# wildjames/lfit_python

Hardware: AMD Instinct MI355X
Metric: walker ln_prob evals/sec (300-pt phase, complex BS) at 1/2/4/8 MI355X (higher is better)
Workload: dtype f64

## Files before the change

cpu_baseline/lfg_cpu.cpp:

```cpp
#include <omp.h>
#include <stdint.h>
#include <stdlib.h>

#include <algorithm>
#include <cmath>
#include <vector>

#include "lfg.h"
#include "lfg_cpu.h"
#include "lfg_device.hpp"
#include "lfg_tables.hpp"

using namespace lfg;

namespace {

constexpr int U_WD = NWD / 2, U_DISC = NDISC / 2, U_DON = NDONOR / 4;

struct Pair {
    Roche R;
    double s, c, rwd_a, rdisc_a, reff, rcal, ulimb, dexp, L, upk, umax, lnpk, exp1, exp2;
    double bsx, bsy, caz, saz, nb0, nb1, nb2, bden, fis, phi0, wdf, df, sf, rsf;
    double inc;
};
// ... 69 lines not shown
    G.bden = p[11] + (1.0 - p[11]) * std::fmax(std::fabs(st_) * G.s + ct_ * G.c, 0.0);
    G.fis = p[11];
    G.phi0 = p[13];
    G.ulimb = p[7];
    G.dexp = p[12];
    G.L = p[9] * R.xl1;
    G.reff = eggleton(R.q);
    const double sce = G.s * std::cos(PI * p[5]);
    G.rcal = std::sqrt(1.0 - sce * sce);
    G.wdf = p[0]; G.df = p[1]; G.sf = p[2]; G.rsf = p[3];
    G.inc = inc;
    return ST_OK;
}

struct Tables {
    double a[NWD + NDISC], b[NWD + NDISC], w[NWD + NDISC];
    int wd[NWD + NDISC];
    double sa[NBS], sb[NBS], sw[NBS];
    double dv[NDONOR][3], dcen[NDONOR], dhw[NDONOR];
    double dnorm;
};

#ifdef LFC_COUNT
static unsigned long long g_cnt[4 + 3 * 8];
extern "C" void lfc_counts(unsigned long long* o) { for (int i = 0; i < 4 + 24; ++i) o[i] = g_cnt[i]; }
static unsigned long long g_ucost[U_WD + U_DISC + NBS];
extern "C" void lfc_ucost(unsigned long long* o) { for (int i = 0; i < U_WD + U_DISC + NBS; ++i) { o[i] = g_ucost[i]; g_ucost[i] = 0; } }
static void count_pair(const int* cost, int n)
{
    unsigned long long ls = 0, cm = 0, nc = 0;
    for (int k = 0; k < n; k += 64) {
        int m = 0;
        for (int i = k; i < std::min(n, k + 64); ++i) {
            m = std::max(m, cost[i]);
            ls += cost[i];
            const int reg = i < U_WD ? 0 : (i < U_WD + U_DISC ? 1 : 2);
#pragma omp atomic
            g_ucost[i] += cost[i];
#pragma omp atomic
            g_cnt[4 + reg * 8 + std::min(cost[i], 7)] += 1;
        }
        cm += m; ++nc;
    }
#pragma omp atomic
    g_cnt[0] += n;
#pragma omp atomic
    g_cnt[1] += ls;
#pragma omp atomic
    g_cnt[2] += nc;
#pragma omp atomic
    g_cnt[3] += cm;
}
static unsigned long long g_cnt2[5];
extern "C" void lfc_counts2(unsigned long long* o) { for (int i = 0; i < 5; ++i) o[i] = g_cnt2[i]; }
static void count2(int i, unsigned long long v)
{
#pragma omp atomic
    g_cnt2[i] += v;
}
#define LFC_NIT int nit[3] = {0, 0, 0}; bool fb = false; double gs[2] = {0.0, 0.0};
#define LFC_NITARGS , &fb, nit, gs
#if LFC_COST_MODE == 1
#define LFC_COST(v) cost[v] = nit[0] / 1000
#else
#define LFC_COST(v) cost[v] = nit[0] % 1000 + std::max(nit[1], nit[2]) + (fb ? 30 : 0); count2(0, nit[0] / 1000); count2(1, fb)
#endif
static std::vector<double> g_ab;
extern "C" long lfc_dump(double* o, long n)
{
    const long m = std::min<long>(n, long(g_ab.size()));
    for (long i = 0; i < m; ++i) o[i] = g_ab[i];
    g_ab.clear();
    return m;
}
#define LFC_AB(a, b) do { _Pragma("omp critical") { g_ab.push_back(a); g_ab.push_back(b); g_gs.push_back(gs[0]); g_gs.push_back(gs[1]); } } while (0)
static std::vector<double> g_gs;
extern "C" long lfc_dump_guess(double* o, long n)
{
    const long m = std::min<long>(n, long(g_gs.size()));
    for (long i = 0; i < m; ++i) o[i] = g_gs[i];
    g_gs.clear();
    return m;
}
#else
#define LFC_NIT
#define LFC_NITARGS
#define LFC_COST(v)
#define LFC_AB(a, b)
#endif

void elements(const Pair& G, Tables& T)
{
#ifdef LFC_COUNT
    int cost[U_WD + U_DISC + NBS] = {0};
#endif
    const Roche& R = G.R;
    const double s = G.s, c = G.c;
    const double twd = TWO_PI * ((1.0 - G.ulimb) * 0.5 + G.ulimb / 3.0);
    const double td = TWO_PI * (disc_boundary(NDISC_R, G) - disc_boundary(0, G));
    int k = 0;
    for (int u = 0; u < U_WD + U_DISC; ++u) {
        double Px, Py, Pz, wgt;
        bool isw = u < U_WD;
        if (isw) {
            const int ir = wd_ring_of(u);
            const double rc = kWdRc[ir], mu0 = kWdMu0[ir], cp = kWdCos[u], sp = kWdSin[u];
            Px = G.rwd_a * (-rc * sp * c + mu0 * s);
            Py = G.rwd_a * (rc * cp);
            Pz = G.rwd_a * (rc * sp * s + mu0 * c);
            wgt = std::fma(kWdA[ir], 1.0 - G.ulimb, kWdB[ir] * G.ulimb) / twd;
        } else {
            const int uu = u - U_WD, ir = uu / (NDISC_AZ / 2), j = uu - ir * (NDISC_AZ / 2);
            const double rc = G.rwd_a + (ir + 0.5) * ((G.rdisc_a - G.rwd_a) / NDISC_R);
            Px = rc * kDiscCos[j];
            Py = rc * kDiscSin[j];
            Pz = 0.0;
            wgt = (TWO_PI / NDISC_AZ) * (disc_boundary(ir + 1, G) - disc_boundary(ir, G)) / td;
        }
        double a, b;
        LFC_NIT
        element_interval_fast(R, Px, Py, Pz, s, c, G.rcal, G.reff, a, b LFC_NITARGS);
        LFC_COST(u);
        LFC_AB(a, b);
        T.a[k] = a; T.b[k] = b; T.w[k] = wgt; T.wd[k] = isw; ++k;
        const bool ecl = a < b;
        T.a[k] = ecl ? -b : 1.0; T.b[k] = ecl ? -a : -1.0; T.w[k] = wgt; T.wd[k] = isw; ++k;
    }
    double tot = 0.0;
    for (int j = 0; j < NBS; ++j) {
        const double uk = (j + 0.5) * (G.umax / NBS);
        T.sw[j] = std::exp(G.exp1 * std::log(uk) - std::pow(uk, G.exp2) - G.lnpk);
        tot += T.sw[j];
        const double off = G.L * (uk - G.upk);
        LFC_NIT
        element_interval_fast(R, std::fma(off, G.caz, G.bsx), std::fma(off, G.saz, G.bsy), 0.0, s, c, G.rcal, G.reff,
                              T.sa[j], T.sb[j] LFC_NITARGS);
        LFC_COST(U_WD + U_DISC + j);
        LFC_AB(T.sa[j], T.sb[j]);
    }
#ifdef LFC_COUNT
    count_pair(cost, U_WD + U_DISC + NBS);
#endif
    for (int j = 0; j < NBS; ++j) T.sw[j] /= tot;
    double dn = 0.0;
    for (int uu = 0; uu < U_DON; ++uu) {
        const int it = uu / (NDONOR_P / 4), ip = uu - it * (NDONOR_P / 4);
        const double dx = -kDonCt[it], dy = kDonSt[it] * kDonCp[ip], dz = kDonSt[it] * kDonSp[ip];
        double lo = 0.0, hi = R.Rs, r = G.reff, gx, gy, gz;
        if (!(r > lo && r < hi)) r = 0.5 * hi;
#if LFG_F32_OPEN && LFG_F32_ROOT_STEPS > 0
        r = root_open32<LFG_F32_ROOT_STEPS>(R, dx, dy, dz, hi, r);
#endif
#ifdef LFC_COUNT
        count2(2, 1);
        count2(4, LFG_F32_OPEN ? LFG_F32_ROOT_STEPS : 0);
#endif
        for (int itr = 0; itr < ROOT_MAXIT; ++itr) {
#ifdef LFC_COUNT
            count2(3, 1);
#endif
            const double f = rpot_grad(R, std::fma(r, dx, 1.0), r * dy, r * dz, gx, gy, gz) - R.pl1;
            const double df = gx * dx + gy * dy + gz * dz;
            if (f > 0.0) hi = r; else lo = r;
            if (df > 0.0 && std::fabs(f / df) <= ROOT_LAST) { r -= f / df; break; }
            double rn = (df > 0.0) ? r - f / df : 0.5 * (lo + hi);
            if (!(rn > lo && rn < hi)) rn = 0.5 * (lo + hi);
// ... 430 lines not shown
```

cpu_baseline/shim/hip/hip_runtime.h:

```cpp
#pragma once
#include <algorithm>
#include <cmath>
#define __device__
#define __host__
#define __global__
#define __constant__
#define __forceinline__ inline
#define __noinline__
#define __builtin_amdgcn_rsq(x) (1.0 / std::sqrt(x))
#define __builtin_amdgcn_rcp(x) (1.0 / (x))
#define __builtin_amdgcn_rsqf(x) (1.0f / std::sqrt(float(x)))
#define __builtin_amdgcn_rcpf(x) (1.0f / float(x))
using std::max;
using std::min;
inline double rsqrt(double x) { return 1.0 / std::sqrt(x); }
inline float rsqrtf(float x) { return 1.0f / std::sqrt(x); }
```

lfit_python_amd/csrc/lfg_device.hpp:

```cpp
#pragma once
#include <hip/hip_runtime.h>
#include <math.h>

#include "lfg_stream_table.h"

namespace lfg {

constexpr double PI = 3.14159265358979323846;
constexpr double TWO_PI = 6.28318530717958647693;
constexpr double DEG = PI / 180.0;
constexpr double LN2 = 0.69314718055994530942;

constexpr double RAY_TOL = 1e-13;
constexpr int RAY_MAXIT = 100;
constexpr double TH_TOL = 1e-13;
constexpr int ROOT_MAXIT = 100;
constexpr double ROOT_LAST = 1e-9;
constexpr int MIN_MAXIT = 100;
constexpr double BS_TAIL = 16.0;
constexpr double STREAM_DELTA = 1e-2;
constexpr double STREAM_KAPPA_FINE = 0.15 / 32.0;
constexpr double STREAM_DTMAX_FINE = 0.15 / 32.0;
constexpr int STREAM_MAXSTEP_FINE = 128000;
constexpr double DISC_MAX_A = 0.46;
constexpr double AZ_SLOPE = 80.0;
constexpr double DPHI_TOL = 1e-6;

constexpr int NWD_RINGS = 10;
constexpr int NWD = 400;
constexpr int NDISC_R = 20;
constexpr int NDISC_AZ = 50;
constexpr int NDISC = 1000;
constexpr int NBS = 100;
constexpr int NDONOR_T = 20;
constexpr int NDONOR_P = 20;
constexpr int NDONOR = 400;
constexpr int NEL = NWD + NDISC + NBS;
constexpr int NALL = NEL + NDONOR;

enum Status { ST_OK = 0, ST_BAD_Q = 1, ST_BAD_DPHI = 2, ST_BAD_GEOMETRY = 3,
              ST_BAD_STREAM = 4, ST_BAD_ARGS = 5 };

enum Geo {
    G_Q, G_CA, G_CB, G_MU, G_XL1, G_PL1, G_RS, G_RS2,
    G_S, G_C, G_INC, G_RWD, G_RDISC, G_REFF, G_ULIMB, G_DEXP,
    G_BSX, G_BSY, G_BSVX, G_BSVY, G_L, G_UPK, G_UMAX, G_LNPK,
    G_EXP1, G_EXP2, G_CAZ, G_SAZ, G_NB0, G_NB1, G_NB2, G_BDEN,
    G_FIS, G_PHI0, G_WDF, G_DF, G_SF, G_RSF, G_RPRIOR, G_RCAL,
    G_RPRIOR_BS,
    G_GP_AIN, G_GP_AOUT, G_GP_LAM, G_GP_DCP, G_GP_OK,
    G_GP_DPHI, G_GP_RWD,
    G_COUNT
};
static_assert(G_COUNT <= 48, "LFG_NGEO");

struct Roche {
    double q, cA, cB, mu, xl1, pl1, Rs, Rs2;
};

__device__ __forceinline__ double rsqrt_pos(double x)
{
    const double y = __builtin_amdgcn_rsq(x);
    const double e = fma(-x * y, y, 1.0);
    return fma(y * e, fma(e, 0.375, 0.5), y);
}

__device__ __forceinline__ double rcp_fast(double x)
{
    const double y = __builtin_amdgcn_rcp(x);
    return fma(y, fma(-x, y, 1.0), y);
}

__device__ __forceinline__ double rcp_step(double x)
{
    return __builtin_amdgcn_rcp(x);
}

__device__ __forceinline__ double rpot(const Roche& R, double x, double y, double z)
{
    const double dx = x - 1.0;
    const double xc = x - R.mu;
    return -R.cA * rsqrt(x * x + y * y + z * z) - R.cB * rsqrt(dx * dx + y * y + z * z)
           - xc * xc - y * y;
}

__device__ __forceinline__ double rpot_grad(const Roche& R, double x, double y, double z, double& gx, double& gy,
                                            double& gz)
// ... 195 lines not shown
    const double Dm = (cosD <= -1.0) ? PI : acos(cosD);
    const double lo = thc - Dm, hi = thc + Dm;

    double tw = -1.0, g, dg;
    bool chord = g_eval(R, Px, Py, Pz, s, c, thc, tw, g, dg);
    if (!chord) return false;
    double thi = thc;
    if (!(g < 0.0)) {
        bool found = false, have = false;
        double th = thc, pth = 0.0, pdg = 0.0, mlo = lo, mhi = hi;
        for (int it = 0; it < MIN_MAXIT; ++it) {
            if (chord) {
                if (g < 0.0) { found = true; thi = th; break; }
                if (dg > 0.0) mhi = th; else mlo = th;
            } else {
                if (th < thc) mlo = th; else mhi = th;
            }
            double tn = (chord && have && dg != pdg) ? th - dg * (th - pth) / (dg - pdg)
                                                     : 0.5 * (mlo + mhi);
            if (!(tn > mlo && tn < mhi)) tn = 0.5 * (mlo + mhi);
            if (fabs(tn - th) <= TH_TOL) break;
            if (chord) { pth = th; pdg = dg; have = true; }
            th = tn;
            chord = g_eval(R, Px, Py, Pz, s, c, th, tw, g, dg);
        }
        if (!found) return false;
    }
    double de;
    const double ce = (sqrt(fmax(uu - Reff * Reff, 0.0)) - c * uz) / (s * uxy);
    de = (ce > -1.0 && ce < 1.0) ? acos(ce) : 0.5 * Dm;
    double twi = tw, two = tw;
    const double thin = theta_root(R, Px, Py, Pz, s, c, lo, thi, true, thc - de, twi);
    const double thout = theta_root(R, Px, Py, Pz, s, c, thi, hi, false, thc + de, two);
    a = thin * (1.0 / TWO_PI);
    b = thout * (1.0 / TWO_PI);
    return true;
}

struct ConePt {
    double phi, gth, F2, eHe, etHe, ethHeth, gtt, dX2;
};

__device__ __forceinline__ void cone_point(const Roche& R, double Px, double Py, double Pz, double s,
                                           double c, double cs, double sn, double t, ConePt& o)
{
    const double ex = s * cs, ey = -s * sn;
    const double x = fma(t, ex, Px), y = fma(t, ey, Py), z = fma(t, c, Pz);
    const double r1s = x * x + y * y + z * z;
    const double ir1 = rsqrt_pos(r1s), ir1s = ir1 * ir1;
    const double dx = x - 1.0;
    const double r2s = dx * dx + y * y + z * z;
    const double ir2 = rsqrt_pos(r2s), ir2s = ir2 * ir2;
    const double i1 = R.cA * ir1s * ir1, i2 = R.cB * ir2s * ir2, i12 = i1 + i2;
    const double xm = x - R.mu;
    o.phi = -R.cA * ir1 - R.cB * ir2 - xm * xm - y * y;
    const double gx = i1 * x + i2 * dx - 2.0 * xm;
    const double gy = (i12 - 2.0) * y;
    const double gz = i12 * z;
    const double p1 = x * ex + y * ey + z * c, p2 = p1 - ex;
    const double q1 = x * ey - y * ex, q2 = q1 - ey;
    const double k1 = 3.0 * i1 * ir1s, k2 = 3.0 * i2 * ir2s;
    const double s2 = ex * ex + ey * ey;
    o.F2 = gx * ex + gy * ey + gz * c;
    o.gth = gx * ey - gy * ex;
    o.eHe = i12 - k1 * p1 * p1 - k2 * p2 * p2 - 2.0 * s2;
    o.etHe = -k1 * p1 * q1 - k2 * p2 * q2;
    o.ethHeth = i12 * s2 - k1 * q1 * q1 - k2 * q2 * q2 - 2.0 * s2;
    o.gtt = -(gx * ex + gy * ey);
    o.dX2 = r2s;
}

__device__ __forceinline__ void rotate(double& cs, double& sn, double d)
{
    const double d2 = d * d;
    const double sd = d * (1.0 - d2 * (1.0 / 6.0) * (1.0 - d2 * (1.0 / 20.0) * (1.0 - d2 * (1.0 / 42.0) *
                                                                              (1.0 - d2 * (1.0 / 72.0)))));
    const double cd = 1.0 - d2 * 0.5 * (1.0 - d2 * (1.0 / 12.0) * (1.0 - d2 * (1.0 / 30.0) *
                                                                    (1.0 - d2 * (1.0 / 56.0) * (1.0 - d2 * (1.0 / 90.0)))));
    const double c2 = cs * cd - sn * sd;
    sn = fma(sn, cd, cs * sd);
    cs = c2;
}

#ifndef LFG_TH_LAST
#define LFG_TH_LAST 1e-6
#endif
#ifndef LFG_T_LAST
#define LFG_T_LAST 3e-5
#endif
constexpr double TH_LAST = LFG_TH_LAST;
constexpr double T_LAST = LFG_T_LAST;

struct Tan {
    double th, cs, sn, t;
    int st;
};

template <bool HALLEY = false>
__device__ __forceinline__ void tangency_step(const Roche& R, double Px, double Py, double Pz, double s, double c,
                                              bool ingress, Tan& T, bool halley = true)
{
    ConePt o;
    cone_point(R, Px, Py, Pz, s, c, T.cs, T.sn, T.t, o);
    const double F1 = o.phi - R.pl1;
    const double J11 = T.t * o.gth;
    const double J21 = T.t * o.etHe + o.gth, J22 = o.eHe;
    const double iJ22 = rcp_step(J22);
    const double dt0 = -o.F2 * iJ22;
    const double F1m = fma(0.5 * o.F2, dt0, F1);
    const double den = fma(J21, dt0, J11);
    const bool bad = !(J22 != 0.0) || !(den != 0.0);
    const double iden = rcp_step(den);
    double dth = -F1m * iden;
    if (HALLEY && halley) {
        const double g2 = fma(T.t, fma(T.t, o.ethHeth, o.gtt), -J21 * J21 * iJ22);
        const double h = 0.5 * dth * g2 * iden;
        if (fabs(h) < 0.5) dth = dth * rcp_step(1.0 + h);
    }
    dth = fmin(fmax(dth, -0.05), 0.05);
    const double dt = fma(-J21 * iJ22, dth, dt0);
    T.th += dth;
    T.t += dt;
    const bool conv = fabs(dth) <= TH_LAST && fabs(dt) <= T_LAST;
    const bool good = J22 > 0.0 && ((J11 < 0.0) == ingress) && T.t > 0.0 && o.dX2 < R.Rs2;
    rotate(T.cs, T.sn, dth);
    T.st = bad ? -1 : (conv ? (good ? 1 : -1) : 0);
}

__device__ inline bool tangency(const Roche& R, double Px, double Py, double Pz, double s, double c,
                                bool ingress, double& th, double cs, double sn, double& t, int* nit = nullptr)
{
    Tan T{th, cs, sn, t, 0};
    for (int it = 0; it < 16 && T.st == 0; ++it) {
        if (nit) ++*nit;
        tangency_step(R, Px, Py, Pz, s, c, ingress, T);
    }
    th = T.th;
    t = T.t;
    return T.st == 1;
}

__device__ inline void tangency_pair(const Roche& R, double Px, double Py, double Pz, double s, double c, Tan& A,
                                     Tan& B, int* nit = nullptr, bool halleyA = true, bool halleyB = true)
{
    tangency_step<true>(R, Px, Py, Pz, s, c, true, A, halleyA);
    tangency_step<true>(R, Px, Py, Pz, s, c, false, B, halleyB);
    if (nit) { nit[0] += 1; nit[1] += 1; }
    if (A.st != 0 && B.st != 0) return;
    for (int it = 1; it < 16; ++it) {
        Tan A2 = A, B2 = B;
        tangency_step(R, Px, Py, Pz, s, c, true, A2);
        tangency_step(R, Px, Py, Pz, s, c, false, B2);
        if (nit) { nit[0] += (A.st == 0); nit[1] += (B.st == 0); }
        if (A.st == 0) A = A2;
        if (B.st == 0) B = B2;
        if (A.st != 0 && B.st != 0) break;
    }
}

__device__ __forceinline__ void ray_min_prestep(const Roche& R, double Px, double Py, double Pz, double s, double c,
                                                double icb, Tan& T)
{
    const double ex = s * T.cs, ey = -s * T.sn;
    const double x = fma(T.t, ex, Px), y = fma(T.t, ey, Py), z = fma(T.t, c, Pz);
    const double ir1 = rsqrt_pos(x * x + y * y + z * z), ir1s = ir1 * ir1;
    const double eX = x * ex + y * ey + z * c;
    const double i1 = R.cA * ir1s * ir1;
    const double slope = fma(i1, eX, -2.0 * fma(x - R.mu, ex, y * ey));
    const double curv = fma(i1, fma(-3.0 * eX * eX, ir1s, 1.0), icb);
    T.t -= slope * rcp_fast(curv);
}

#ifndef LFG_F32_OPEN
#define LFG_F32_OPEN 1
#endif
#ifndef LFG_F32_STEPS
#define LFG_F32_STEPS 2
#endif
#ifndef LFG_F32_NEWTON_AFTER
#define LFG_F32_NEWTON_AFTER 1
#endif
#ifndef LFG_F32_ROOT_STEPS
#define LFG_F32_ROOT_STEPS 0
#endif

#if LFG_F32_OPEN
constexpr float F32_OPEN_MIN_WIDTH = 0.03f;
#ifdef __HIP__
typedef float F2 __attribute__((ext_vector_type(2)));
#else
struct F2 {
    float x, y;
};
inline F2 operator+(F2 a, F2 b) { return F2{a.x + b.x, a.y + b.y}; }
inline F2 operator-(F2 a, F2 b) { return F2{a.x - b.x, a.y - b.y}; }
inline F2 operator*(F2 a, F2 b) { return F2{a.x * b.x, a.y * b.y}; }
inline F2 operator-(F2 a) { return F2{-a.x, -a.y}; }
#endif
__device__ __forceinline__ F2 f2(float a) { return F2{a, a}; }
__device__ __forceinline__ F2 f2_rsq(F2 a) { return F2{__builtin_amdgcn_rsqf(a.x), __builtin_amdgcn_rsqf(a.y)}; }
__device__ __forceinline__ F2 f2_rcp(F2 a) { return F2{__builtin_amdgcn_rcpf(a.x), __builtin_amdgcn_rcpf(a.y)}; }

template <int N>
__device__ __forceinline__ void tangency_open32(const Roche& R, double Px, double Py, double Pz, double s, double c,
                                                double Rcal, Tan& A, Tan& B, bool& okA, bool& okB)
{
    float dA, dB, tA, tB;
    okA = okB = true;
    {
        const float cA = float(R.cA), cB = float(R.cB), mu = float(R.mu), pl1 = float(R.pl1);
        const F2 px = f2(float(Px)), py = f2(float(Py)), pz = f2(float(Pz)), sf = f2(float(s)), cf = f2(float(c));
        const float rc = float(Rcal);
        const F2 icb = f2(cB * __builtin_amdgcn_rcpf(rc * rc * rc)) - f2(2.0f) * sf * sf;
        F2 cs{float(A.cs), float(B.cs)}, sn{float(A.sn), float(B.sn)}, t{float(A.t), float(B.t)};
        F2 sum = f2(0.0f);
        {
            const F2 ex = sf * cs, ey = -(sf * sn);
            const F2 x = t * ex + px, y = t * ey + py, z = t * cf + pz;
            const F2 ir1 = f2_rsq(x * x + y * y + z * z), ir1s = ir1 * ir1;
            const F2 eX = x * ex + y * ey + z * cf;
            const F2 i1 = f2(cA) * ir1s * ir1;
            const F2 slope = i1 * eX - f2(2.0f) * ((x - f2(mu)) * ex + y * ey);
            const F2 curv = i1 * (f2(1.0f) - f2(3.0f) * eX * eX * ir1s) + icb;
            t = t - slope * f2_rcp(curv);
        }
#pragma unroll
        for (int k = 0; k < N; ++k) {
            const F2 ex = sf * cs, ey = -(sf * sn);
            const F2 x = t * ex + px, y = t * ey + py, z = t * cf + pz;
            const F2 yz = y * y + z * z;
            const F2 ir1 = f2_rsq(x * x + yz), ir1s = ir1 * ir1;
            const F2 dx = x - f2(1.0f);
            const F2 ir2 = f2_rsq(dx * dx + yz), ir2s = ir2 * ir2;
            const F2 i1 = f2(cA) * ir1s * ir1, i2 = f2(cB) * ir2s * ir2, i12 = i1 + i2;
            const F2 xm = x - f2(mu);
            const F2 F1 = -(f2(cA) * ir1) - f2(cB) * ir2 - xm * xm - y * y - f2(pl1);
            const F2 gx = i1 * x + i2 * dx - f2(2.0f) * xm;
            const F2 gy = (i12 - f2(2.0f)) * y;
            const F2 gz = i12 * z;
            const F2 p1 = x * ex + y * ey + z * cf, p2 = p1 - ex;
            const F2 q1 = x * ey - y * ex, q2 = q1 - ey;
            const F2 k1 = f2(3.0f) * i1 * ir1s, k2 = f2(3.0f) * i2 * ir2s;
            const F2 s2 = ex * ex + ey * ey;
            const F2 Ft = gx * ex + gy * ey + gz * cf;
            const F2 gth = gx * ey - gy * ex;
            const F2 J22 = i12 - k1 * p1 * p1 - k2 * p2 * p2 - f2(2.0f) * s2;
            const F2 etHe = -(k1 * p1 * q1) - k2 * p2 * q2;
            const F2 J11 = t * gth, J21 = t * etHe + gth;
            const F2 iJ22 = f2_rcp(J22);
            const F2 dt0 = -(Ft * iJ22);
            const F2 F1m = f2(0.5f) * Ft * dt0 + F1;
            const F2 iden = f2_rcp(J21 * dt0 + J11);
            F2 dth = -(F1m * iden);
            if (k == 0) {
                const F2 ethHeth = i12 * s2 - k1 * q1 * q1 - k2 * q2 * q2 - f2(2.0f) * s2;
                const F2 gtt = -(gx * ex + gy * ey);
                const F2 g2 = t * (t * ethHeth + gtt) - J21 * J21 * iJ22;
                const F2 h = f2(0.5f) * dth * g2 * iden;
                const F2 dh = dth * f2_rcp(f2(1.0f) + h);
                dth = F2{fabsf(h.x) < 0.5f ? dh.x : dth.x, fabsf(h.y) < 0.5f ? dh.y : dth.y};
            }
            okA = okA && J22.x > 0.0f && fabsf(dth.x) <= 0.05f;
            okB = okB && J22.y > 0.0f && fabsf(dth.y) <= 0.05f;
            t = t + (dt0 - J21 * iJ22 * dth);
            sum = sum + dth;
            const F2 d2 = dth * dth;
            const F2 sd = dth * (f2(1.0f) - d2 * f2(1.0f / 6.0f) * (f2(1.0f) - d2 * f2(1.0f / 20.0f)));
            const F2 cd = f2(1.0f) - d2 * f2(0.5f) * (f2(1.0f) - d2 * f2(1.0f / 12.0f) *
                                                                  (f2(1.0f) - d2 * f2(1.0f / 30.0f)));
            const F2 c2 = cs * cd - sn * sd;
            sn = sn * cd + cs * sd;
            cs = c2;
        }
        const bool wide = float(B.th - A.th) + (sum.y - sum.x) >= F32_OPEN_MIN_WIDTH;
        okA = okA && wide && fabsf(sum.x) <= 0.05f && t.x > 0.0f && t.x < 3.0e38f;
        okB = okB && wide && fabsf(sum.y) <= 0.05f && t.y > 0.0f && t.y < 3.0e38f;
        dA = okA ? sum.x : 0.0f;
        dB = okB ? sum.y : 0.0f;
        tA = t.x;
        tB = t.y;
    }
    A.th += double(dA);
    B.th += double(dB);
    rotate(A.cs, A.sn, double(dA));
    rotate(B.cs, B.sn, double(dB));
    A.t = double(tA);
    B.t = double(tB);
    if (!(okA && okB)) {
        const double icb = R.cB / (Rcal * Rcal * Rcal) - 2.0 * s * s;
        for (int k = 0; k < 2; ++k) {
            Tan& T = k ? B : A;
            if (k ? okB : okA) continue;
            T.t = s * ((1.0 - Px) * T.cs + Py * T.sn) - Pz * c;
            ray_min_prestep(R, Px, Py, Pz, s, c, icb, T);
        }
    }
}

template <int N>
__device__ __forceinline__ double root_open32(const Roche& R, double dx, double dy, double dz, double hi, double r0)
{
    const float cA = float(R.cA), cB = float(R.cB), mu = float(R.mu), pl1 = float(R.pl1);
    const float ax = float(dx), ay = float(dy), az = float(dz), top = float(hi);
    float r = float(r0);
    bool ok = true;
#pragma unroll
    for (int k = 0; k < N; ++k) {
        const float x = fmaf(r, ax, 1.0f), y = r * ay, z = r * az, x1 = r * ax;
        const float yz = y * y + z * z;
        const float ir1 = __builtin_amdgcn_rsqf(x * x + yz), ir2 = __builtin_amdgcn_rsqf(x1 * x1 + yz);
        const float i1 = cA * ir1 * ir1 * ir1, i2 = cB * ir2 * ir2 * ir2;
        const float xm = x - mu;
        const float f = -cA * ir1 - cB * ir2 - xm * xm - y * y - pl1;
        const float gx = i1 * x + i2 * x1 - 2.0f * xm, gy = (i1 + i2 - 2.0f) * y, gz = (i1 + i2) * z;
        const float df = gx * ax + gy * ay + gz * az;
        r -= f * __builtin_amdgcn_rcpf(df);
        ok = ok && df > 0.0f && r > 0.0f && r < top;
    }
    return ok ? double(r) : r0;
}
#endif

__device__ inline int cone_exists(const Roche& R, double Px, double Py, double Pz, double s, double c,
                                  double cs, double sn, double t, int* nit = nullptr)
{
    for (int it = 0; it < 16; ++it) {
        if (nit) ++*nit;
        ConePt o;
        cone_point(R, Px, Py, Pz, s, c, cs, sn, t, o);
        if (o.phi < R.pl1) return (o.dX2 < R.Rs2) ? 1 : -1;
        const double Gth = t * o.gth, Gt = o.F2;
        const double Htt = o.eHe, Hht = o.gth + t * o.etHe, Hhh = t * t * o.ethHeth + t * o.gtt;
        const double det = Hhh * Htt - Hht * Hht;
        if (!(Hhh > 0.0 && Htt > 0.0 && det > 0.0)) return -1;
        const double idet = rcp_fast(det);
        double dth = -(Htt * Gth - Hht * Gt) * idet;
        double dt = -(Hhh * Gt - Hht * Gth) * idet;
        const double big = fmax(fabs(dth), fabs(dt));
        if (big > 0.05) {
            dth *= 0.05 / big;
            dt *= 0.05 / big;
        }
        t += dt;
        if (fabs(dth) <= 1e-12 && fabs(dt) <= 1e-12) return 0;
        rotate(cs, sn, dth);
    }
    return -1;
}

__device__ inline bool element_interval_fast(const Roche& R, double Px, double Py, double Pz, double s,
                                             double c, double Rcal, double Reff, double& a, double& b,
                                             bool* fallback = nullptr, int* nit = nullptr, double* guess = nullptr)
{
    const double ux = 1.0 - Px, uy = -Py, uz = -Pz;
    const double uxy2 = ux * ux + uy * uy;
    const double uu = uxy2 + uz * uz;
    if (uu > R.Rs2 && uxy2 > 0.0 && s > 0.0) {
        const double iuxy = rsqrt(uxy2), uxy = uxy2 * iuxy;
        const double cosD = (sqrt(uu - R.Rs2) - c * uz) * iuxy / s;
        if (!(cosD < 1.0)) { a = 1.0; b = -1.0; return false; }
        const double cc = ux * iuxy, sc = -uy * iuxy;
        const double tc = s * uxy + uz * c;
        int ex;
        {
            const double ex0 = s * cc, ey0 = -s * sc;
            const double x = fma(tc, ex0, Px), y = fma(tc, ey0, Py), z = fma(tc, c, Pz);
            const double dx = x - 1.0, xm = x - R.mu;
            const double r2s = dx * dx + y * y + z * z;
            const double phi = -R.cA * rsqrt_pos(x * x + y * y + z * z) - R.cB * rsqrt_pos(r2s) - xm * xm - y * y;
            if (phi < R.pl1 && r2s < R.Rs2) {
                ex = 1;
                if (nit) ++nit[0];
            } else {
                ex = cone_exists(R, Px, Py, Pz, s, c, cc, sc, tc, nit);
            }
        }
        if (ex == 0) { a = 1.0; b = -1.0; return false; }
        if (ex == 1) {
            const double ce = (sqrt(fmax(uu - Rcal * Rcal, 0.0)) - c * uz) * iuxy / s;
            if (ce > -1.0 && ce < 1.0) {
                const double se = sqrt(1.0 - ce * ce);
                const double thc = atan2(-uy, ux), de = acos(ce);
                double ci = cc * ce + sc * se, si = sc * ce - cc * se;
                double co = cc * ce - sc * se, so = sc * ce + cc * se;
                Tan In{thc - de, ci, si, s * (ux * ci - uy * si) + uz * c, 0};
                Tan Out{thc + de, co, so, s * (ux * co - uy * so) + uz * c, 0};
                if (guess) { guess[0] = In.th; guess[1] = Out.th; }
#if LFG_F32_OPEN
                bool openIn, openOut;
                tangency_open32<LFG_F32_STEPS>(R, Px, Py, Pz, s, c, Rcal, In, Out, openIn, openOut);
                if (nit) nit[0] += 1000 * LFG_F32_STEPS;
                const bool hIn = !(LFG_F32_NEWTON_AFTER && openIn), hOut = !(LFG_F32_NEWTON_AFTER && openOut);
#else
                {
                    const double icb = R.cB / (Rcal * Rcal * Rcal) - 2.0 * s * s;
                    for (Tan* T : {&In, &Out}) ray_min_prestep(R, Px, Py, Pz, s, c, icb, *T);
                }
#endif
#if LFG_F32_OPEN
                tangency_pair(R, Px, Py, Pz, s, c, In, Out, nit ? nit + 1 : nullptr, hIn, hOut);
#else
                tangency_pair(R, Px, Py, Pz, s, c, In, Out, nit ? nit + 1 : nullptr);
#endif
                const double cin = In.cs * cc + In.sn * sc, cout = Out.cs * cc + Out.sn * sc;
                if (In.st == 1 && Out.st == 1 && In.th < Out.th && cin > cosD && cout > cosD) {
                    a = In.th * (1.0 / TWO_PI);
                    b = Out.th * (1.0 / TWO_PI);
                    return true;
                }
            }
        }
    }
    if (fallback) *fallback = true;
    return element_interval(R, Px, Py, Pz, s, c, Reff, a, b);
}

__device__ inline int findphi(const Roche& R, double inc_deg, double& dphi);

__device__ inline int findphi_fast(const Roche& R, double inc_deg, double& dphi)
{
    double s, c;
    sincos(inc_deg * DEG, &s, &c);
    const double cosD = sqrt(1.0 - R.Rs2) / s;
    if (s > 0.0 && cosD < 1.0) {
        const double Dm = acos(cosD);
        const double R0 = eggleton(R.q);
        const double c0 = sqrt(1.0 - R0 * R0) / s;
        double th = (c0 < 1.0) ? acos(c0) : 0.5 * Dm;
        double sn, cs;
        sincos(th, &sn, &cs);
        double t = s * cs;
        if (tangency(R, 0.0, 0.0, 0.0, s, c, false, th, cs, sn, t) && th > 0.0 && th < Dm) {
            dphi = th / PI;
            return ST_OK;
        }
    }
    return findphi(R, inc_deg, dphi);
}

__device__ inline int findphi(const Roche& R, double inc_deg, double& dphi)
{
    const double i = inc_deg * DEG;
    double s, c;
    sincos(i, &s, &c);
    dphi = 0.0;
    const double cosD = sqrt(1.0 - R.Rs2) / s;
    if (!(s > 0.0) || cosD >= 1.0) return ST_BAD_DPHI;
    const double Dm = acos(cosD);
    double tw = -1.0, g, dg;
    g_eval(R, 0.0, 0.0, 0.0, s, c, 0.0, tw, g, dg);
    if (!(g < 0.0)) return ST_BAD_DPHI;
    const double th = theta_root(R, 0.0, 0.0, 0.0, s, c, 0.0, Dm, false, 0.5 * Dm, tw);
    dphi = th / PI;
    return ST_OK;
}

__device__ inline bool h_eval(const Roche& R, double cth, double sth, double c,
                              double& tw, double& h, double& dh)
{
    const double s = sqrt(1.0 - c * c);
    const double ex = s * cth, ey = -s * sth;
    double fm;
    if (!ray_min(R, 0.0, 0.0, 0.0, ex, ey, c, tw, fm)) { h = 1.0; dh = 0.0; return false; }
    double gx, gy, gz;
    rgrad(R, tw * ex, tw * ey, tw * c, gx, gy, gz);
    h = fm - R.pl1;
    const double r = c / s;
    dh = tw * (gx * (-r * cth) + gy * (r * sth) + gz);
    return true;
}

__device__ inline int findi(const Roche& R, double dphi, double& inc_deg)
{
    if (!(dphi > 0.0) || !(dphi < 0.5)) return ST_BAD_DPHI;
    const double the = PI * dphi;
    double sth, cth;
    sincos(the, &sth, &cth);
    if (!(cth > 0.0)) return ST_BAD_DPHI;
    const double smin = sqrt(1.0 - R.Rs2) / cth;
    if (smin >= 1.0) return ST_BAD_DPHI;
    const double cmax = sqrt(1.0 - smin * smin);
    double tw = -1.0, h, dh;
    h_eval(R, cth, sth, 0.0, tw, h, dh);
    if (!(h < 0.0)) return ST_BAD_DPHI;
    double lo = 0.0, hi = cmax, c = 0.5 * cmax;
    for (int it = 0; it < ROOT_MAXIT; ++it) {
        h_eval(R, cth, sth, c, tw, h, dh);
        if (h > 0.0) hi = c; else lo = c;
        double cn = (dh != 0.0) ? c - h / dh : 0.5 * (lo + hi);
        if (!(cn > lo && cn < hi)) cn = 0.5 * (lo + hi);
        const double d = cn - c;
        c = cn;
        if (fabs(d) <= TH_TOL) break;
    }
// ... 528 lines not shown
```

lfit_python_amd/csrc/lfg_tables.hpp:

```cpp
#pragma once
#include <hip/hip_runtime.h>
namespace lfg {
__constant__ const double kWdCos[200] = {
    0.70710678118654757, 0.70710678118654735, 0.96592582628906831, 0.70710678118654757,
    0.25881904510252074, 0.2588190451025203, 0.70710678118654735, 0.96592582628906809,
    0.98768834059513777, 0.8910065241883679, 0.70710678118654757, 0.4539904997395468,
    0.15643446504023092, 0.15643446504023067, 0.45399049973954664, 0.70710678118654735,
    0.89100652418836779, 0.98768834059513766, 0.9937122098932426, 0.94388333030836757,
    0.84672419922828412, 0.70710678118654757, 0.53203207651533657, 0.33027906195516732,
    0.11196447610330769, 0.11196447610330768, 0.33027906195516687, 0.53203207651533635,
    0.70710678118654735, 0.84672419922828401, 0.94388333030836746, 0.9937122098932426,
    0.99619469809174555, 0.96592582628906831, 0.90630778703664994, 0.8191520442889918,
    0.70710678118654757, 0.57357643635104616, 0.42261826174069944, 0.25881904510252096,
    0.087155742747658138, 0.087155742747657888, 0.2588190451025203, 0.42261826174069883,
    0.57357643635104605, 0.70710678118654735, 0.81915204428899158, 0.90630778703664971,
    0.96592582628906831, 0.99619469809174555, 0.99745211461025352, 0.97714686597115952,
    0.9369497249997617, 0.87767898956725565, 0.80054124092436041, 0.70710678118654757,
    0.59927766651134695, 0.479248986720057, 0.34946417959909842, 0.21256528955297682,
    0.071339183199232353, 0.071339183199231673, 0.21256528955297679, 0.34946417959909837,
    0.47924898672005678, 0.59927766651134684, 0.70710678118654735, 0.80054124092436019,
    0.87767898956725543, 0.93694972499976192, 0.97714686597115941, 0.99745211461025352,
    0.9981755542233175, 0.98361990694714363, 0.9547208665085456, 0.91189984599209006,
    0.85578127230144752, 0.7871834806090503, 0.70710678118654746, 0.61671887262854319,
    0.51733781417765679, 0.41041280545275693, 0.29750305385520298, 0.18025503781390587,
// ... 74 lines not shown
    0.93159108805127899, 0.9584274824582526, 0.97871684532735448, 0.99232057973704502,
    0.99914575838730102, -0.99914575838730102, -0.99232057973704513, -0.97871684532735448,
    -0.9584274824582526, -0.9315910880512791, -0.89839098189197897, -0.85905395436988519,
    -0.81384871727019537, -0.76308406819980623, -0.70710678118654768, -0.64629923786094157,
    -0.58107681540193812, -0.51188504908960131, -0.43919658884737051, -0.36350797056382977,
    -0.28533622424910587, -0.20521534219563378, -0.12369263126934776, -0.041324974248814018};
__constant__ const double kWdRc[10] = {
    0.070710678118654766, 0.15811388300841897, 0.25495097567963926, 0.35355339059327379,
    0.45276925690687087, 0.55226805085936304, 0.65192024052026487, 0.75166481891864545,
    0.85146931829632011, 0.95131487952202243};
__constant__ const double kWdMu0[10] = {
    0.99749686716300012, 0.98742088290657493, 0.9669539802906858, 0.93541434669348533,
    0.89162772500635035, 0.83366660002665338, 0.758287544405155, 0.65954529791364591,
    0.5244044240850757, 0.30822070014844877};
__constant__ const double kWdA[10] = {
    0.0078539816339744835, 0.0078539816339744835, 0.0078539816339744817, 0.007853981633974487,
    0.00785398163397448, 0.0078539816339744817, 0.00785398163397448, 0.0078539816339744922,
    0.00785398163397448, 0.00785398163397448};
__constant__ const double kWdB[10] = {
    0.0078343138316304111, 0.0077551089948375658, 0.0075942125464331647, 0.0073462371702575054,
    0.0070018923404746164, 0.0065458916079624389, 0.0059523977588250079, 0.0051736044474914276,
    0.004101962746066755, 0.0022823141497946139};
__constant__ const unsigned char kWdRingOf[400] = {
    0, 0, 0, 0, 1, 1, 1, 1, 1, 1, 1, 1, 1, 1, 1, 1, 2, 2, 2, 2,
    2, 2, 2, 2, 2, 2, 2, 2, 2, 2, 2, 2, 2, 2, 2, 2, 3, 3, 3, 3,
    3, 3, 3, 3, 3, 3, 3, 3, 3, 3, 3, 3, 3, 3, 3, 3, 3, 3, 3, 3,
    3, 3, 3, 3, 4, 4, 4, 4, 4, 4, 4, 4, 4, 4, 4, 4, 4, 4, 4, 4,
    4, 4, 4, 4, 4, 4, 4, 4, 4, 4, 4, 4, 4, 4, 4, 4, 4, 4, 4, 4,
    5, 5, 5, 5, 5, 5, 5, 5, 5, 5, 5, 5, 5, 5, 5, 5, 5, 5, 5, 5,
    5, 5, 5, 5, 5, 5, 5, 5, 5, 5, 5, 5, 5, 5, 5, 5, 5, 5, 5, 5,
    5, 5, 5, 5, 6, 6, 6, 6, 6, 6, 6, 6, 6, 6, 6, 6, 6, 6, 6, 6,
    6, 6, 6, 6, 6, 6, 6, 6, 6, 6, 6, 6, 6, 6, 6, 6, 6, 6, 6, 6,
    6, 6, 6, 6, 6, 6, 6, 6, 6, 6, 6, 6, 6, 6, 6, 6, 7, 7, 7, 7,
    7, 7, 7, 7, 7, 7, 7, 7, 7, 7, 7, 7, 7, 7, 7, 7, 7, 7, 7, 7,
    7, 7, 7, 7, 7, 7, 7, 7, 7, 7, 7, 7, 7, 7, 7, 7, 7, 7, 7, 7,
    7, 7, 7, 7, 7, 7, 7, 7, 7, 7, 7, 7, 7, 7, 7, 7, 8, 8, 8, 8,
    8, 8, 8, 8, 8, 8, 8, 8, 8, 8, 8, 8, 8, 8, 8, 8, 8, 8, 8, 8,
    8, 8, 8, 8, 8, 8, 8, 8, 8, 8, 8, 8, 8, 8, 8, 8, 8, 8, 8, 8,
    8, 8, 8, 8, 8, 8, 8, 8, 8, 8, 8, 8, 8, 8, 8, 8, 8, 8, 8, 8,
    8, 8, 8, 8, 9, 9, 9, 9, 9, 9, 9, 9, 9, 9, 9, 9, 9, 9, 9, 9,
    9, 9, 9, 9, 9, 9, 9, 9, 9, 9, 9, 9, 9, 9, 9, 9, 9, 9, 9, 9,
    9, 9, 9, 9, 9, 9, 9, 9, 9, 9, 9, 9, 9, 9, 9, 9, 9, 9, 9, 9,
    9, 9, 9, 9, 9, 9, 9, 9, 9, 9, 9, 9, 9, 9, 9, 9, 9, 9, 9, 9};
__constant__ const double kDiscCos[25] = {
    0.99802672842827156, 0.98228725072868872, 0.95105651629515353, 0.90482705246601958,
    0.84432792550201508, 0.77051324277578925, 0.68454710592868862, 0.58778525229247325,
    0.48175367410171516, 0.36812455268467809, 0.24868988716485474, 0.12533323356430448,
    6.123233995736766e-17, -0.12533323356430415, -0.24868988716485485, -0.36812455268467775,
    -0.48175367410171543, -0.58778525229247303, -0.68454710592868873, -0.77051324277578914,
    -0.84432792550201485, -0.90482705246601935, -0.95105651629515353, -0.98228725072868872,
    -0.99802672842827156};
__constant__ const double kDiscSin[25] = {
    0.062790519529313374, 0.1873813145857246, 0.3090169943749474, 0.42577929156507266,
    0.53582679497899666, 0.63742398974868963, 0.72896862742141155, 0.80901699437494734,
    0.87630668004386369, 0.92977648588825135, 0.96858316112863108, 0.99211470131447776,
    1, 0.99211470131447788, 0.96858316112863108, 0.92977648588825146,
    0.87630668004386347, 0.80901699437494745, 0.72896862742141144, 0.63742398974868986,
    0.53582679497899699, 0.42577929156507288, 0.30901699437494751, 0.18738131458572457,
    0.062790519529313582};
__constant__ const double kDonCt[20] = {
    0.99691733373312796, 0.97236992039767656, 0.92387953251128674, 0.85264016435409218,
    0.76040596560003093, 0.64944804833018366, 0.52249856471594891, 0.38268343236508984,
    0.23344536385590547, 0.078459095727844999, -0.078459095727844874, -0.23344536385590534,
    -0.38268343236508973, -0.5224985647159488, -0.64944804833018355, -0.76040596560003093,
    -0.85264016435409218, -0.92387953251128674, -0.97236992039767656, -0.99691733373312796};
__constant__ const double kDonSt[20] = {
    0.078459095727844944, 0.23344536385590539, 0.38268343236508978, 0.5224985647159488,
    0.64944804833018366, 0.76040596560003093, 0.85264016435409218, 0.92387953251128674,
    0.97236992039767656, 0.99691733373312796, 0.99691733373312796, 0.97236992039767667,
    0.92387953251128674, 0.85264016435409229, 0.76040596560003104, 0.64944804833018377,
    0.52249856471594891, 0.38268343236508989, 0.23344536385590553, 0.078459095727845068};
__constant__ const double kDonOmega[20] = {
    0.0038678218739814866, 0.011508227010842255, 0.01886526140508028, 0.0257577704533123,
    0.032016037707844669, 0.037485963858872651, 0.04203286117091376, 0.045544769941858576,
    0.047935215322409457, 0.04914533661386386, 0.049145336613863791, 0.047935215322409526,
    0.045544769941858576, 0.04203286117091376, 0.037485963858872651, 0.032016037707844669,
    0.0257577704533123, 0.018865261405080314, 0.011508227010842221, 0.0038678218739815213};
__constant__ const double kDonCp[5] = {
    0.98768834059513777, 0.8910065241883679, 0.70710678118654757, 0.4539904997395468,
    0.15643446504023092};
__constant__ const double kDonSp[5] = {
    0.15643446504023087, 0.45399049973954675, 0.70710678118654746, 0.89100652418836779,
    0.98768834059513777};
}
```

Before: 14.19 million.

## Compute tangency start guesses in float32 and rebuild directions from a sin/cos table

The single-tangency (ex==1) start path now computes the ingress/egress guess angles and ray parameters in float32. It runs the float32 open-tangency refinement on those guesses directly, and rebuilds the double-precision cos/sin of the refined angles from an 81-entry table plus a Taylor rotation instead of calling double sincos. The aim is to replace costly double-precision transcendentals (atan2, acos, sincos) in the per-element start. The trade-off is start guesses of lower precision and a hard |theta|<=5 domain limit. The old path is kept behind LFG_TAB_START=0, and a CPU test hook is added.

After: 14.70 million (median of 6 runs). 1.04x the previous value.

```diff
diff --git a/cpu_baseline/lfg_cpu.cpp b/cpu_baseline/lfg_cpu.cpp
--- a/cpu_baseline/lfg_cpu.cpp
+++ b/cpu_baseline/lfg_cpu.cpp
@@ -175,6 +175,10 @@
     g_gs.clear();
     return m;
 }
+extern "C" void lfc_unit_dir(const double* th, long n, double* cs, double* sn, int* ok)
+{
+    for (long i = 0; i < n; ++i) ok[i] = unit_dir(th[i], cs[i], sn[i]) ? 1 : 0;
+}
 #else
 #define LFC_NIT
 #define LFC_NITARGS
diff --git a/cpu_baseline/shim/hip/hip_runtime.h b/cpu_baseline/shim/hip/hip_runtime.h
--- a/cpu_baseline/shim/hip/hip_runtime.h
+++ b/cpu_baseline/shim/hip/hip_runtime.h
@@ -11,6 +11,7 @@
 #define __builtin_amdgcn_rcp(x) (1.0 / (x))
 #define __builtin_amdgcn_rsqf(x) (1.0f / std::sqrt(float(x)))
 #define __builtin_amdgcn_rcpf(x) (1.0f / float(x))
+#define __builtin_amdgcn_sqrtf(x) std::sqrt(float(x))
 using std::max;
 using std::min;
 inline double rsqrt(double x) { return 1.0 / std::sqrt(x); }
diff --git a/lfit_python_amd/csrc/lfg_device.hpp b/lfit_python_amd/csrc/lfg_device.hpp
--- a/lfit_python_amd/csrc/lfg_device.hpp
+++ b/lfit_python_amd/csrc/lfg_device.hpp
@@ -3,6 +3,7 @@
 #include <math.h>
 
 #include "lfg_stream_table.h"
+#include "lfg_tables.hpp"
 
 namespace lfg {
 
@@ -364,6 +365,23 @@
     cs = c2;
 }
 
+#ifndef LFG_TAB_START
+#define LFG_TAB_START 1
+#endif
+constexpr double UNIT_MAX = 5.0;
+static_assert(sizeof(kUnitCos) / sizeof(double) == 81 && sizeof(kUnitSin) / sizeof(double) == 81, "UNIT_MAX * 16 + 1");
+
+__device__ __forceinline__ bool unit_dir(double th, double& cs, double& sn)
+{
+    if (!(fabs(th) <= UNIT_MAX)) return false;
+    const double kf = rint(th * 16.0);
+    const int k = min(int(fabs(kf)), 80);
+    cs = kUnitCos[k];
+    sn = kf < 0.0 ? -kUnitSin[k] : kUnitSin[k];
+    rotate(cs, sn, fma(kf, -0.0625, th));
+    return true;
+}
+
 #ifndef LFG_TH_LAST
 #define LFG_TH_LAST 1e-6
 #endif
@@ -484,17 +502,16 @@
 __device__ __forceinline__ F2 f2_rcp(F2 a) { return F2{__builtin_amdgcn_rcpf(a.x), __builtin_amdgcn_rcpf(a.y)}; }
 
 template <int N>
-__device__ __forceinline__ void tangency_open32(const Roche& R, double Px, double Py, double Pz, double s, double c,
-                                                double Rcal, Tan& A, Tan& B, bool& okA, bool& okB)
-{
-    float dA, dB, tA, tB;
+__device__ __forceinline__ void tangency_open32_steps(const Roche& R, double Px, double Py, double Pz, double s,
+                                                      double c, double Rcal, F2 cs, F2 sn, F2 t, float width,
+                                                      float& dA, float& dB, float& tA, float& tB, bool& okA, bool& okB)
+{
     okA = okB = true;
     {
         const float cA = float(R.cA), cB = float(R.cB), mu = float(R.mu), pl1 = float(R.pl1);
         const F2 px = f2(float(Px)), py = f2(float(Py)), pz = f2(float(Pz)), sf = f2(float(s)), cf = f2(float(c));
         const float rc = float(Rcal);
         const F2 icb = f2(cB * __builtin_amdgcn_rcpf(rc * rc * rc)) - f2(2.0f) * sf * sf;
-        F2 cs{float(A.cs), float(B.cs)}, sn{float(A.sn), float(B.sn)}, t{float(A.t), float(B.t)};
         F2 sum = f2(0.0f);
         {
             const F2 ex = sf * cs, ey = -(sf * sn);
@@ -554,7 +571,7 @@
             sn = sn * cd + cs * sd;
             cs = c2;
         }
-        const bool wide = float(B.th - A.th) + (sum.y - sum.x) >= F32_OPEN_MIN_WIDTH;
+        const bool wide = width + (sum.y - sum.x) >= F32_OPEN_MIN_WIDTH;
         okA = okA && wide && fabsf(sum.x) <= 0.05f && t.x > 0.0f && t.x < 3.0e38f;
         okB = okB && wide && fabsf(sum.y) <= 0.05f && t.y > 0.0f && t.y < 3.0e38f;
         dA = okA ? sum.x : 0.0f;
@@ -562,6 +579,16 @@
         tA = t.x;
         tB = t.y;
     }
+}
+
+#if !LFG_TAB_START
+template <int N>
+__device__ __forceinline__ void tangency_open32(const Roche& R, double Px, double Py, double Pz, double s, double c,
+                                                double Rcal, Tan& A, Tan& B, bool& okA, bool& okB)
+{
+    float dA, dB, tA, tB;
+    tangency_open32_steps<N>(R, Px, Py, Pz, s, c, Rcal, F2{float(A.cs), float(B.cs)}, F2{float(A.sn), float(B.sn)},
+                             F2{float(A.t), float(B.t)}, float(B.th - A.th), dA, dB, tA, tB, okA, okB);
     A.th += double(dA);
     B.th += double(dB);
     rotate(A.cs, A.sn, double(dA));
@@ -578,6 +605,7 @@
         }
     }
 }
+#endif
 
 template <int N>
 __device__ __forceinline__ double root_open32(const Roche& R, double dx, double dy, double dz, double hi, double r0)
@@ -658,6 +686,54 @@
             }
         }
         if (ex == 0) { a = 1.0; b = -1.0; return false; }
+#if LFG_TAB_START
+        if (ex == 1) {
+            const float pxf = float(Px), pyf = float(Py), pzf = float(Pz), sf = float(s), cf = float(c);
+            const float rcf = float(Rcal);
+            const float uxf = 1.0f - pxf, uxy2f = uxf * uxf + pyf * pyf, uuf = uxy2f + pzf * pzf;
+            const float iuf = __builtin_amdgcn_rsqf(uxy2f);
+            const float ccf = uxf * iuf, scf = pyf * iuf;
+            const float cef = (__builtin_amdgcn_sqrtf(fmaxf(uuf - rcf * rcf, 0.0f)) + cf * pzf) * iuf *
+                              __builtin_amdgcn_rcpf(sf);
+            if (cef > -1.0f && cef < 1.0f) {
+                const float sef = __builtin_amdgcn_sqrtf(1.0f - cef * cef);
+                const float thcf = atan2f(scf, ccf), def = acosf(cef);
+                const float thi = thcf - def, tho = thcf + def;
+                const float ci = ccf * cef + scf * sef, si = scf * cef - ccf * sef;
+                const float co = ccf * cef - scf * sef, so = scf * cef + ccf * sef;
+                const float ti = sf * (uxf * ci + pyf * si) - pzf * cf, to = sf * (uxf * co + pyf * so) - pzf * cf;
+                if (guess) { guess[0] = double(thi); guess[1] = double(tho); }
+                float dIn = 0.0f, dOut = 0.0f, tIn = 0.0f, tOut = 0.0f;
+                bool openIn = false, openOut = false;
+#if LFG_F32_OPEN
+                tangency_open32_steps<LFG_F32_STEPS>(R, Px, Py, Pz, s, c, Rcal, F2{ci, co}, F2{si, so}, F2{ti, to},
+                                                     tho - thi, dIn, dOut, tIn, tOut, openIn, openOut);
+                if (nit) nit[0] += 1000 * LFG_F32_STEPS;
+#endif
+                Tan In{double(thi) + double(dIn), 1.0, 0.0, double(tIn), 0};
+                Tan Out{double(tho) + double(dOut), 1.0, 0.0, double(tOut), 0};
+                if (unit_dir(In.th, In.cs, In.sn) && unit_dir(Out.th, Out.cs, Out.sn)) {
+                    if (!(openIn && openOut)) {
+                        const double icb = R.cB / (Rcal * Rcal * Rcal) - 2.0 * s * s;
+                        for (int k = 0; k < 2; ++k) {
+                            Tan& T = k ? Out : In;
+                            if (k ? openOut : openIn) continue;
+                            T.t = s * (ux * T.cs - uy * T.sn) + uz * c;
+                            ray_min_prestep(R, Px, Py, Pz, s, c, icb, T);
+                        }
+                    }
+                    const bool hIn = !(LFG_F32_NEWTON_AFTER && openIn), hOut = !(LFG_F32_NEWTON_AFTER && openOut);
+                    tangency_pair(R, Px, Py, Pz, s, c, In, Out, nit ? nit + 1 : nullptr, hIn, hOut);
+                    const double cin = In.cs * cc + In.sn * sc, cout = Out.cs * cc + Out.sn * sc;
+                    if (In.st == 1 && Out.st == 1 && In.th < Out.th && cin > cosD && cout > cosD) {
+                        a = In.th * (1.0 / TWO_PI);
+                        b = Out.th * (1.0 / TWO_PI);
+                        return true;
+                    }
+                }
+            }
+        }
+#else
         if (ex == 1) {
             const double ce = (sqrt(fmax(uu - Rcal * Rcal, 0.0)) - c * uz) * iuxy / s;
             if (ce > -1.0 && ce < 1.0) {
@@ -692,6 +768,7 @@
                 }
             }
         }
+#endif
     }
     if (fallback) *fallback = true;
     return element_interval(R, Px, Py, Pz, s, c, Reff, a, b);
diff --git a/lfit_python_amd/csrc/lfg_tables.hpp b/lfit_python_amd/csrc/lfg_tables.hpp
--- a/lfit_python_amd/csrc/lfg_tables.hpp
+++ b/lfit_python_amd/csrc/lfg_tables.hpp
@@ -180,4 +180,48 @@
 __constant__ const double kDonSp[5] = {
     0.15643446504023087, 0.45399049973954675, 0.70710678118654746, 0.89100652418836779,
     0.98768834059513777};
+__constant__ const double kUnitCos[81] = {
+    1, 0.99804751070009912, 0.99219766722932901, 0.9824733131012553,
+    0.96891242171064473, 0.95156794804817224, 0.93050762191231429, 0.90581368342593638,
+    0.87758256189037276, 0.84592449923106794, 0.81096311950521793, 0.7728349461524715,
+    0.7316888688738209, 0.68768556222050481, 0.64099685816332508, 0.59180507509247748,
+    0.54030230586813977, 0.48668966770196331, 0.4311765167986662, 0.37397963082453317,
+    0.31532236239526867, 0.2554337668888117, 0.19454770798898718, 0.13290194445282522,
+    0.070737201667702906, 0.0082962316238583775, -0.054177135026936322, -0.11643894112485226,
+    -0.17824605564949209, -0.2393571231413216, -0.29953350618957414, -0.35854021730623281,
+    -0.41614683654714241, -0.4721284112969602, -0.52626633470430506, -0.57834919933683349,
+    -0.62817362272273913, -0.67554504155495254, -0.72027847145669177, -0.76219922934149464,
+    -0.8011436155469337, -0.83695955307829428, -0.86950718146598438, -0.89865940291767599,
+    -0.92430237863246356, -0.94633597333894548, -0.96467414632131632, -0.9792452874065205,
+    -0.98999249660044542, -0.9968738062811815, -0.99986234508168659, -0.99894644282190015,
+    -0.99412967608054625, -0.98543085422866994, -0.97288394597944639, -0.9565379467410825,
+    -0.93645668729079634, -0.9127185845169985, -0.88541633520302043, -0.85465655404815977,
+    -0.82055935733956076, -0.78325789390068368, -0.74289782514799874, -0.69963675628627164,
+    -0.65364362086361194, -0.60509802108958288, -0.55418952649241671, -0.50111693365406351,
+    -0.44608748991379282, -0.38931608407176954, -0.3310244072528874, -0.27144008720767066,
+    -0.2107957994307797, -0.14932835856818344, -0.087277793661034928, -0.024886410837402149,
+    0.037602152887976553, 0.099943881011021238, 0.16189533041753676, 0.22321458202336397,
+    0.28366218546322625};
+__constant__ const double kUnitSin[81] = {
+    0, 0.062459317842380201, 0.12467473338522769, 0.18640329676226988,
+    0.24740395925452294, 0.30743851458038085, 0.36627252908604757, 0.42367625720393803,
+    0.47942553860420301, 0.53330267353602012, 0.58509727294046221, 0.63460708001526933,
+    0.68163876002333412, 0.72600865526071257, 0.76754350223602708, 0.80608110826069301,
+    0.8414709848078965, 0.87357493516707108, 0.90226759409909518, 0.92743691738486767,
+    0.9489846193555862, 0.96682655669618023, 0.98089305702315566, 0.99112919095376162,
+    0.99749498660405445, 0.99996558567824889, 0.99853134053983161, 0.9931978518853749,
+    0.98398594687393692, 0.97093159779745053, 0.95408578160969382, 0.9335142808623762,
+    0.90929742682568171, 0.8815297857963782, 0.85031978981845202, 0.81578931325829696,
+    0.7780731968879212, 0.73731872133461895, 0.6936850319532718, 0.64734251736714443,
+    0.59847214410395655, 0.54726474992546525, 0.49392029861008918, 0.43864709909863309,
+    0.38166099205233167, 0.32318450699968687, 0.26344599336342084, 0.20267872876086712,
+    0.14112000805986721, 0.079010216747389686, 0.016591892229347906, -0.045891223272779696,
+    -0.10819513453010837, -0.17007654610249431, -0.23129381240202182, -0.2916078813138529,
+    -0.35078322768961984, -0.40858877306808949, -0.46479878803160896, -0.51919377367465125,
+    -0.57156131874234373, -0.62169692909187302, -0.66940482623773601, -0.71449871186253666,
+    -0.7568024953079282, -0.79615098120486583, -0.83239051455798729, -0.86537958076508192,
+    -0.8949893582285835, -0.92110422140115222, -0.94362219230096245, -0.96245533873353939,
+    -0.97753011766509701, -0.98878766240651084, -0.99618401248647925, -0.99969028531622339,
+    -0.99929278897537799, -0.99499307567864759, -0.98680793571444114, -0.97476933187915538,
+    -0.95892427466313845};
 }
```
